# ParBLiSS/FastANI

Measured on AMD Instinct MI355X. Metric: ANI pairs/sec, many-to-many NxN ~5 Mbp genomes, higher is better.
Workload: dtype u32

## Files before the change

### fastani_amd/csrc/kernels/common.hpp

```cpp
#pragma once
#include <hip/hip_runtime.h>
#include <stdint.h>

#if defined(__HIP_DEVICE_COMPILE__)
#define ANI_CONSUME(x) asm volatile("" : "+v"(x))
#else
#define ANI_CONSUME(x) (void)(x)
#endif

namespace ani {

constexpr int kWave = 64;
constexpr int kTPB = 256;
constexpr uint32_t kMurmurSeed = 42;
constexpr uint32_t kSingleNone = 0xffffffffu;

constexpr int kStatStripes = 32;
constexpr int kStatStripeWords = 24;
__device__ __forceinline__ unsigned long long *stat_slot(unsigned long long *base) { return base + (blockIdx.x & (kStatStripes - 1)) * kStatStripeWords; }

constexpr int kPoolStripes = 64, kPoolStripeWords = 16;
constexpr unsigned long long kPoolOverflowBit = 1ull << 63;
__device__ __forceinline__ unsigned long long pool_take(unsigned long long *cursors, uint32_t stripeCap, unsigned long long n)
{
  const uint32_t r = blockIdx.x & (kPoolStripes - 1);
  const unsigned long long off = n ? atomicAdd(&cursors[r * kPoolStripeWords], n) : 0ull;
  return ((unsigned long long)r * stripeCap + off) | (off + n > (unsigned long long)stripeCap ? kPoolOverflowBit : 0ull);
}

__host__ __device__ __forceinline__ uint64_t rotl64(uint64_t x, int r)
{
#if defined(__HIP_DEVICE_COMPILE__)
  uint32_t lo = (uint32_t)x, hi = (uint32_t)(x >> 32);
  if (r >= 32) { const uint32_t t = lo; lo = hi; hi = t; r -= 32; }
  if (r == 0) return ((uint64_t)hi << 32) | lo;
  const uint32_t nh = __builtin_amdgcn_alignbit(hi, lo, 32 - r), nl = __builtin_amdgcn_alignbit(lo, hi, 32 - r);
  return ((uint64_t)nh << 32) | nl;
#else
  return (x << r) | (x >> (64 - r));
#endif
}

__host__ __device__ __forceinline__ uint64_t xorshr33(uint64_t z)
{
  const uint32_t hi = (uint32_t)(z >> 32);
  return ((uint64_t)hi << 32) | ((uint32_t)z ^ (hi >> 1));
}
__host__ __device__ __forceinline__ uint64_t fmix64(uint64_t z)
{
  z = xorshr33(z); z *= 0xff51afd7ed558ccdULL;
  z = xorshr33(z); z *= 0xc4ceb9fe1a85ec53ULL;
  return xorshr33(z);
}

__host__ __device__ __forceinline__ uint32_t murmur32_k16(uint64_t k1, uint64_t k2)
{
  const uint64_t c1 = 0x87c37b91114253d5ULL, c2 = 0x4cf5ad432745937fULL;
  uint64_t h1 = kMurmurSeed, h2 = kMurmurSeed;
  k1 *= c1; k1 = rotl64(k1, 31); k1 *= c2; h1 ^= k1;
  h1 = rotl64(h1, 27); h1 += h2; h1 = h1 * 5 + 0x52dce729;
  k2 *= c2; k2 = rotl64(k2, 33); k2 *= c1; h2 ^= k2;
  h2 = rotl64(h2, 31); h2 += h1; h2 = h2 * 5 + 0x38495ab5;
  h1 ^= 16; h2 ^= 16;
  h1 += h2; h2 += h1;
  h1 = fmix64(h1); h2 = fmix64(h2);
  return (uint32_t)(h1 + h2);
}

__host__ __device__ __forceinline__ uint32_t murmur32_tail(uint64_t k1, uint64_t k2, int k)
{
  const uint64_t c1 = 0x87c37b91114253d5ULL, c2 = 0x4cf5ad432745937fULL;
  uint64_t h1 = kMurmurSeed, h2 = kMurmurSeed;
  if (k > 8) { k2 *= c2; k2 = rotl64(k2, 33); k2 *= c1; h2 ^= k2; }
  k1 *= c1; k1 = rotl64(k1, 31); k1 *= c2; h1 ^= k1;
  h1 ^= (uint64_t)k; h2 ^= (uint64_t)k;
  h1 += h2; h2 += h1;
  h1 = fmix64(h1); h2 = fmix64(h2);
  return (uint32_t)(h1 + h2);
}

__host__ __device__ __forceinline__ uint32_t perm_b32(uint32_t hi, uint32_t lo, uint32_t sel)
{
#if defined(__HIP_DEVICE_COMPILE__)
  return __builtin_amdgcn_perm(hi, lo, sel);
#else
  const uint64_t src = ((uint64_t)hi << 32) | lo;
  uint32_t r = 0;
  for (int i = 0; i < 4; i++) r |= (uint32_t)((src >> (8 * ((sel >> (8 * i)) & 7u))) & 0xffu) << (8 * i);
  return r;
#endif
}
__host__ __device__ __forceinline__ uint32_t alignbyte(uint32_t hi, uint32_t lo, uint32_t n)
{
#if defined(__HIP_DEVICE_COMPILE__)
  return __builtin_amdgcn_alignbyte(hi, lo, n);
#else
  return (uint32_t)(((((uint64_t)hi << 32) | lo) >> (8 * (n & 3u))) & 0xffffffffu);
#endif
}
__host__ __device__ __forceinline__ uint32_t spread_codes4(uint32_t c8)
{
  const uint32_t t = (c8 | (c8 << 12)) & 0x000F000Fu;
  return (t | (t << 6)) & 0x03030303u;
}

__host__ __device__ __forceinline__ uint32_t code_to_ascii(uint32_t c) { return (0x54474341u >> (8 * c)) & 0xffu; }
__host__ __device__ __forceinline__ uint32_t code_to_ascii_comp(uint32_t c) { return (0x41434754u >> (8 * c)) & 0xffu; }
__host__ __device__ __forceinline__ uint32_t ascii_comp(uint32_t b)
{
  return b == 'A' ? 'T' : b == 'C' ? 'G' : b == 'G' ? 'C' : b == 'T' ? 'A' : b;
}
__host__ __device__ __forceinline__ uint32_t ascii_upper(uint32_t b) { return (b > 96 && b < 123) ? b - 32 : b; }

__device__ __forceinline__ int wave_incl_scan(int v)
{
  const int lane = threadIdx.x & (kWave - 1);
#pragma unroll
  for (int d = 1; d < kWave; d <<= 1) {
    int o = __shfl_up(v, d);
    if (lane >= d) v += o;
  }
  return v;
}

__device__ __forceinline__ int wave_incl_scan_dpp(int v)
{
#if defined(__HIP_DEVICE_COMPILE__)
  v += __builtin_amdgcn_update_dpp(0, v, 0x111, 0xf, 0xf, false);
  v += __builtin_amdgcn_update_dpp(0, v, 0x112, 0xf, 0xf, false);
  v += __builtin_amdgcn_update_dpp(0, v, 0x114, 0xf, 0xf, false);
  v += __builtin_amdgcn_update_dpp(0, v, 0x118, 0xf, 0xf, false);
  v += __builtin_amdgcn_update_dpp(0, v, 0x142, 0xa, 0xf, false);
  v += __builtin_amdgcn_update_dpp(0, v, 0x143, 0xc, 0xf, false);
  return v;
#else
  return wave_incl_scan(v);
#endif
}

__device__ __forceinline__ void block_barrier()
{
#if defined(__HIP_DEVICE_COMPILE__)
  asm volatile("s_waitcnt lgkmcnt(0)" ::: "memory");
#endif
  __syncthreads();
}
__device__ __forceinline__ void block_barrier_mem()
{
#if defined(__HIP_DEVICE_COMPILE__)
  asm volatile("s_waitcnt vmcnt(0) lgkmcnt(0)" ::: "memory");
#endif
  __syncthreads();
}

#if defined(__HIP_DEVICE_COMPILE__)
__device__ __forceinline__ uint32_t wave_uniform(uint32_t x) { return (uint32_t)__builtin_amdgcn_readfirstlane((int)x); }
#else
__device__ __forceinline__ uint32_t wave_uniform(uint32_t x) { return x; }
#endif
__device__ __forceinline__ int32_t wave_uniform(int32_t x) { return (int32_t)wave_uniform((uint32_t)x); }
#if defined(__HIP_DEVICE_COMPILE__)
__device__ __forceinline__ int32_t lane_value(int32_t x, int l) { return __builtin_amdgcn_readlane(x, l); }
#else
__device__ __forceinline__ int32_t lane_value(int32_t x, int l) { return __shfl(x, l); }
#endif
__device__ __forceinline__ uint64_t wave_uniform(uint64_t x) { return (uint64_t)wave_uniform((uint32_t)x) | ((uint64_t)wave_uniform((uint32_t)(x >> 32))
    << 32); }

__device__ __forceinline__ int block_excl_scan(int v, int *ws, int *total)
{
  const int lane = threadIdx.x & (kWave - 1), wv = threadIdx.x >> 6;
  int incl = wave_incl_scan(v);
  block_barrier();
  if (lane == kWave - 1) ws[wv] = incl;
  block_barrier();
  int base = 0, tot = 0;
#pragma unroll
  for (int i = 0; i < kTPB / kWave; i++) { int x = ws[i]; if (i < wv) base += x; tot += x; }
  *total = wave_uniform(tot);
  return base + incl - v;
}

__device__ __forceinline__ int block_incl_maxscan(int v, int *ws)
{
  const int lane = threadIdx.x & (kWave - 1), wv = threadIdx.x >> 6;
#pragma unroll
  for (int d = 1; d < kWave; d <<= 1) {
    int o = __shfl_up(v, d);
    if (lane >= d) v = o > v ? o : v;
  }
  block_barrier();
  if (lane == kWave - 1) ws[wv] = v;
  block_barrier();
#pragma unroll
  for (int i = 0; i < kTPB / kWave; i++) { int x = ws[i]; if (i < wv) v = x > v ? x : v; }
  return v;
}

__device__ inline int block_array_excl_scan(int *a, int n, int *ws)
{
  int carry = 0;
  for (int base = 0; base < n; base += kTPB * 8) {
    int first = base + (int)threadIdx.x * 8;
    int loc[8]; int sum = 0;
#pragma unroll
    for (int j = 0; j < 8; j++) { int idx = first + j; int x = idx < n ? a[idx] : 0; loc[j] = sum; sum += x; }
    int tot; int off = block_excl_scan(sum, ws, &tot);
#pragma unroll
    for (int j = 0; j < 8; j++) { int idx = first + j; if (idx < n) a[idx] = carry + off + loc[j]; }
    carry += tot;
  }
  block_barrier_mem();
  return carry;
}

#if defined(__HIP_DEVICE_COMPILE__)
#define ANI_WAVE_SYNC() do { __builtin_amdgcn_fence(__ATOMIC_RELEASE, "wavefront"); __builtin_amdgcn_wave_barrier(); \
    __builtin_amdgcn_fence(__ATOMIC_ACQUIRE, "wavefront"); } while (0)
#else
#define ANI_WAVE_SYNC() (void)__ballot(1)
#endif

template <class K>
__device__ __forceinline__ void bitonic_ce(K &x, K &y, bool up) { if ((x > y) == up) { const K t = x; x = y; y = t; } }

template <class K>
__device__ __forceinline__ void bitonic_quad(K *a, int q, int h, int stride, int size)
{
  const int i0 = ((q & ~(h - 1)) << 2) | (q & (h - 1));
  const bool up = ((i0 & size) == 0);
  K x0 = a[i0], x1 = a[i0 + h], x2 = a[i0 + stride], x3 = a[i0 + stride + h];
  bitonic_ce(x0, x2, up); bitonic_ce(x1, x3, up);
  bitonic_ce(x0, x1, up); bitonic_ce(x2, x3, up);
  a[i0] = x0; a[i0 + h] = x1; a[i0 + stride] = x2; a[i0 + stride + h] = x3;
}

template <class K>
__device__ inline void block_bitonic_sort(K *a, int n2)
{
  constexpr int kWaves = kTPB / kWave;
  const int lane = threadIdx.x & (kWave - 1), wv = threadIdx.x >> 6;
  const int seg = n2 > kWaves * kWave ? n2 / kWaves : n2;
  const bool mine = wv * seg < n2;
  block_barrier();
  for (int size = 2; size <= n2; size <<= 1) {
    int stride = size >> 1;
    while (stride >= 2) {
      const int h = stride >> 1;
      if (stride >= seg) {
        block_barrier();
        for (int q = threadIdx.x; q < (n2 >> 2); q += kTPB) bitonic_quad(a, q, h, stride, size);
        block_barrier();
      } else if (mine) {
        ANI_WAVE_SYNC();
        for (int q = wv * (seg >> 2) + lane; q < (wv + 1) * (seg >> 2); q += kWave) bitonic_quad(a, q, h, stride, size);
      }
      stride >>= 2;
    }
    if (stride == 1) {
      if (seg < 2) {
        block_barrier();
      }
      if (mine) {
        ANI_WAVE_SYNC();
        for (int t = wv * (seg >> 1) + lane; t < (wv + 1) * (seg >> 1); t += kWave) {
          const int lo = 2 * t;
          const bool up = ((lo & size) == 0);
          K x = a[lo], y = a[lo + 1];
          if ((x > y) == up) { a[lo] = y; a[lo + 1] = x; }
        }
      }
    }
  }
  block_barrier();
}

template <int M> __device__ __forceinline__ uint32_t lane_xor(uint32_t x)
{
#if defined(__HIP_DEVICE_COMPILE__)
  if constexpr (M == 1) return (uint32_t)__builtin_amdgcn_mov_dpp((int)x, 0xB1, 0xf, 0xf, true);
  else if constexpr (M == 2) return (uint32_t)__builtin_amdgcn_mov_dpp((int)x, 0x4E, 0xf, 0xf, true);
  else if constexpr (M == 4) {
    int r = __builtin_amdgcn_update_dpp(0, (int)x, 0x104, 0xf, 0x5, false);
    return (uint32_t)__builtin_amdgcn_update_dpp(r, (int)x, 0x114, 0xf, 0xA, false);
  }
  else if constexpr (M == 8) return (uint32_t)__builtin_amdgcn_mov_dpp((int)x, 0x128, 0xf, 0xf, true);
  else if constexpr (M == 16) {
    const auto r = __builtin_amdgcn_permlane16_swap(x, x, false, false);
    return (threadIdx.x & 16) ? r[0] : r[1];
  } else {
    const auto r = __builtin_amdgcn_permlane32_swap(x, x, false, false);
    return (threadIdx.x & 32) ? r[0] : r[1];
  }
#else
  return __shfl_xor(x, M);
#endif
}
template <int M> __device__ __forceinline__ uint64_t lane_xor(uint64_t x)
{
#if !defined(__HIP_DEVICE_COMPILE__)
  return __shfl_xor(x, M);
#endif
  return ((uint64_t)lane_xor<M>((uint32_t)(x >> 32)) << 32) | lane_xor<M>((uint32_t)x);
}

template <class K> __device__ __forceinline__ K sort_pick(K own, K partner, bool keepMin) { return ((partner < own) == keepMin) ? partner : own; }

template <class K, int KPT, int M> __device__ __forceinline__ void sort_lane_stage(K (&k)[KPT], bool keepMin)
{
#pragma unroll
  for (int r = 0; r < KPT; r++) k[r] = sort_pick(k[r], lane_xor<M>(k[r]), keepMin);
}
template <class K, int KPT> __device__ __forceinline__ void sort_thread_merge(K (&k)[KPT], bool up)
{
#pragma unroll
  for (int st = KPT >> 1; st >= 1; st >>= 1)
#pragma unroll
    for (int r = 0; r < KPT; r++)
      if ((r & st) == 0) bitonic_ce(k[r], k[r + st], up);
}

template <class K, int KPT, int WAVES>
__device__ __forceinline__ void block_sort_regs(K *a)
{
  constexpr int NT = kWave * WAVES;
  const int t = threadIdx.x;
  if (WAVES == 1 && t >= kWave) return;
  K k[KPT];
#pragma unroll
  for (int r = 0; r < KPT; r++) k[r] = a[r * NT + t];
  if (WAVES > 1) block_barrier();
#pragma unroll
  for (int size = 2; size <= KPT; size <<= 1)
#pragma unroll
    for (int st = size >> 1; st >= 1; st >>= 1)
#pragma unroll
      for (int r = 0; r < KPT; r++)
        if ((r & st) == 0) bitonic_ce(k[r], k[r + st], size < KPT ? (r & size) == 0 : (t & 1) == 0);
  for (int ts = 2; ts <= NT; ts <<= 1) {
    const bool up = (t & ts) == 0;
    for (int m = ts >> 1; m >= 1; m >>= 1) {
      const bool keepMin = ((t & m) == 0) == up;
      if (WAVES > 1 && m >= kWave) {
#pragma unroll
        for (int r = 0; r < KPT; r++) a[r * NT + t] = k[r];
        block_barrier();
#pragma unroll
        for (int r = 0; r < KPT; r++) k[r] = sort_pick(k[r], a[r * NT + (t ^ m)], keepMin);
        block_barrier();
      } else {
        switch (m) {
          case 32: sort_lane_stage<K, KPT, 32>(k, keepMin); break;
          case 16: sort_lane_stage<K, KPT, 16>(k, keepMin); break;
          case 8: sort_lane_stage<K, KPT, 8>(k, keepMin); break;
          case 4: sort_lane_stage<K, KPT, 4>(k, keepMin); break;
          case 2: sort_lane_stage<K, KPT, 2>(k, keepMin); break;
          default: sort_lane_stage<K, KPT, 1>(k, keepMin); break;
        }
      }
    }
    sort_thread_merge<K, KPT>(k, up);
  }
#pragma unroll
  for (int r = 0; r < KPT; r++) a[t * KPT + r] = k[r];
}

template <class K, int KPT> __device__ __forceinline__ void wave_sort_regs(K (&k)[KPT])
{
  const int lane = threadIdx.x & (kWave - 1);
#pragma unroll
  for (int size = 2; size <= KPT; size <<= 1)
#pragma unroll
    for (int st = size >> 1; st >= 1; st >>= 1)
#pragma unroll
      for (int r = 0; r < KPT; r++)
        if ((r & st) == 0) bitonic_ce(k[r], k[r + st], size < KPT ? (r & size) == 0 : (lane & 1) == 0);
  for (int ts = 2; ts <= kWave; ts <<= 1) {
    const bool up = (lane & ts) == 0;
    for (int m = ts >> 1; m >= 1; m >>= 1) {
      const bool keepMin = ((lane & m) == 0) == up;
      switch (m) {
        case 32: sort_lane_stage<K, KPT, 32>(k, keepMin); break;
        case 16: sort_lane_stage<K, KPT, 16>(k, keepMin); break;
        case 8: sort_lane_stage<K, KPT, 8>(k, keepMin); break;
        case 4: sort_lane_stage<K, KPT, 4>(k, keepMin); break;
        case 2: sort_lane_stage<K, KPT, 2>(k, keepMin); break;
        default: sort_lane_stage<K, KPT, 1>(k, keepMin); break;
      }
    }
    sort_thread_merge<K, KPT>(k, up);
  }
}

constexpr int kBlockSortMax = 4096;
__host__ __device__ __forceinline__ int next_pow2_dev(int n) { int p = 1; while (p < n) p <<= 1; return p; }
template <class K>
__device__ __forceinline__ void block_sort(K *a, int n)
{
  int n2 = next_pow2_dev(n); n2 = n2 < kWave ? kWave : n2;
  for (int i = n + (int)threadIdx.x; i < n2; i += kTPB) a[i] = (K)~(K)0;
#ifdef ANI_SORT_LDS
  block_bitonic_sort<K>(a, n2);
  return;
#endif
  block_barrier();
  switch (n2) {
    case 64: block_sort_regs<K, 1, 1>(a); break;
    case 128: block_sort_regs<K, 2, 1>(a); break;
    case 256: block_sort_regs<K, 4, 1>(a); break;
    case 512: block_sort_regs<K, 2, kTPB / kWave>(a); break;
    case 1024: block_sort_regs<K, 4, kTPB / kWave>(a); break;
    case 2048: block_sort_regs<K, 8, kTPB / kWave>(a); break;
    case 4096: block_sort_regs<K, 16, kTPB / kWave>(a); break;
    default: __builtin_trap();
  }
  block_barrier();
}

__device__ __forceinline__ int xcd_item(int block, int gridBlocks) { return (block & 7) * (gridBlocks >> 3) + (block >> 3); }
__host__ __device__ __forceinline__ unsigned pad8(size_t n) { return (unsigned)((n + 7) / 8 * 8); }

__host__ __device__ __forceinline__ int next_pow2(int n) { int p = 1; while (p < n) p <<= 1; return p; }

}
```

### fastani_amd/csrc/kernels/sketch.hpp

```cpp
#pragma once
#include "common.hpp"

namespace ani {

constexpr int kPer = 12;
constexpr int kTile = kTPB * kPer;
constexpr uint64_t kSkipKey = ~0ull;

struct TileDesc {
  int32_t contig;
  int32_t firstPos;
};
struct TileMeta {
  uint32_t off;
  int32_t cnt;
  int32_t firstP;
  int32_t lastP;
};

__device__ __forceinline__ void hash_positions_packed16(const uint32_t *wds, int32_t len, int32_t i0, int local0, uint64_t (&key)[kPer])
{
  const int32_t nWords = (len + 15) >> 4;
  const int32_t w0 = i0 >> 4;
  const int sh = (i0 & 15) * 2;
  const uint64_t a = w0 < nWords ? wds[w0] : 0u, b = w0 + 1 < nWords ? wds[w0 + 1] : 0u, c = w0 + 2 < nWords ? wds[w0 + 2] : 0u;
  const uint64_t lo = a | (b << 32);
  const uint64_t bits = sh ? ((lo >> sh) | (c << (64 - sh))) : lo;
  uint32_t F[7], R[7];
#pragma unroll
  for (int d = 0; d < 7; d++) {
    const uint32_t c8 = (uint32_t)(bits >> (8 * d)) & 0xffu;
    const uint32_t sp = spread_codes4(c8);
    F[d] = perm_b32(0u, 0x54474341u, sp);
    R[6 - d] = perm_b32(0u, 0x41434754u, perm_b32(0u, sp, 0x00010203u));
  }
  const int32_t nPos = len - 16 + 1;
#pragma unroll
  for (int j = 0; j < kPer; j++) {
    uint32_t f[4], r[4];
    const int fq = j >> 2, fr = j & 3, rq = (12 - j) >> 2, rr = (12 - j) & 3;
#pragma unroll
    for (int t = 0; t < 4; t++) {
      f[t] = fr ? alignbyte(F[fq + t + 1], F[fq + t], (uint32_t)fr) : F[fq + t];
      r[t] = rr ? alignbyte(R[rq + t + 1], R[rq + t], (uint32_t)rr) : R[rq + t];
    }
    const uint32_t hf = murmur32_k16(((uint64_t)f[1] << 32) | f[0], ((uint64_t)f[3] << 32) | f[2]);
    const uint32_t hb = murmur32_k16(((uint64_t)r[1] << 32) | r[0], ((uint64_t)r[3] << 32) | r[2]);
    const bool ok = (i0 + j < nPos) && (hf != hb);
    const uint32_t h = hf < hb ? hf : hb;
    key[j] = ok ? (((uint64_t)h << 32) | (uint32_t)(kTile - 1 - (local0 + j))) : kSkipKey;
  }
}

template <bool PACKED>
__device__ __forceinline__ void hash_positions(const void *seq, int64_t off, int32_t len, int32_t i0, int local0,
                                               int k, uint64_t (&key)[kPer])
{
  if (PACKED && k == 16) { hash_positions_packed16((const uint32_t *)seq + off, len, i0, local0, key); return; }
  uint64_t bits = 0;
  const uint8_t *bytes = nullptr;
  if (PACKED) {
    const uint32_t *wds = (const uint32_t *)seq + off;
    const int32_t nWords = (len + 15) >> 4;
    const int32_t w0 = i0 >> 4;
    const int sh = (i0 & 15) * 2;
    uint64_t a = w0 < nWords ? wds[w0] : 0u;
    uint64_t b = w0 + 1 < nWords ? wds[w0 + 1] : 0u;
    uint64_t c = w0 + 2 < nWords ? wds[w0 + 2] : 0u;
    uint64_t lo = a | (b << 32);
    bits = sh ? ((lo >> sh) | (c << (64 - sh))) : lo;
  } else {
    bytes = (const uint8_t *)seq + off;
  }
  auto fwd_byte = [&](int j) -> uint64_t {
    if (PACKED) return code_to_ascii((uint32_t)(bits >> (2 * j)) & 3u);
    int32_t p = i0 + j;
    return p < len ? ascii_upper(bytes[p]) : 0u;
  };
  auto rc_byte = [&](int j) -> uint64_t {
    if (PACKED) return code_to_ascii_comp((uint32_t)(bits >> (2 * j)) & 3u);
    int32_t p = i0 + j;
    return p < len ? ascii_comp(ascii_upper(bytes[p])) : 0u;
  };

  uint64_t flo = 0, fhi = 0, rlo = 0, rhi = 0;
#pragma unroll
  for (int j = 0; j < 8; j++) {
    flo |= fwd_byte(j) << (8 * j);
    fhi |= fwd_byte(8 + j) << (8 * j);
    rhi |= rc_byte(j) << (8 * (7 - j));
    rlo |= rc_byte(8 + j) << (8 * (7 - j));
  }
  const bool k16 = (k == 16);
  const uint64_t maskLo = k >= 8 ? ~0ull : ((1ull << (8 * k)) - 1);
  const uint64_t maskHi = k16 ? ~0ull : (k > 8 ? ((1ull << (8 * (k - 8))) - 1) : 0ull);
  const int rsh = 8 * (16 - k);
  const int32_t nPos = len - k + 1;

#pragma unroll
  for (int j = 0; j < kPer; j++) {
    uint32_t hf, hb;
    if (k16) {
      hf = murmur32_k16(flo, fhi);
      hb = murmur32_k16(rlo, rhi);
    } else {
      uint64_t r1, r2;
      if (rsh < 64) { r1 = (rlo >> rsh) | (rhi << (64 - rsh)); r2 = rhi >> rsh; }
      else { r1 = rsh == 64 ? rhi : (rhi >> (rsh - 64)); r2 = 0; }
      hf = murmur32_tail(flo & maskLo, fhi & maskHi, k);
      hb = murmur32_tail(r1, r2, k);
    }
    const bool ok = (i0 + j < nPos) && (hf != hb);
    const uint32_t h = hf < hb ? hf : hb;
    key[j] = ok ? (((uint64_t)h << 32) | (uint32_t)(kTile - 1 - (local0 + j))) : kSkipKey;
    const uint64_t nb = fwd_byte(16 + j), nc = rc_byte(16 + j);
    flo = (flo >> 8) | (fhi << 56);
    fhi = (fhi >> 8) | (nb << 56);
    rhi = (rhi << 8) | (rlo >> 56);
    rlo = (rlo << 8) | nc;
  }
}

__device__ __forceinline__ void tile_winnow_keys(const uint64_t (&key)[kPer], int32_t B, int32_t nPos, int w, int lo, int hiEmit,
                                                 uint64_t *keys, int *ws,
                                                 uint64_t (&W)[kPer], bool (&em)[kPer], int &tileFirstP, int &tileLastP)
{
  const int t = threadIdx.x;
  const int local0 = t * kPer;
  bool own_ok[kPer];
  if (t == 0) ws[kTPB + 8] = -1;
  if (w >= kPer && w <= 4 * kPer) {
    uint64_t suf = kSkipKey, pre = kSkipKey;
#pragma unroll
    for (int j = kPer - 1; j >= 0; j--) { suf = key[j] < suf ? key[j] : suf; keys[local0 + j] = suf; }
#pragma unroll
    for (int j = 0; j < kPer; j++) { own_ok[j] = key[j] != kSkipKey; pre = key[j] < pre ? key[j] : pre; W[j] = pre; }
    block_barrier();
    const int aHi = (w - 1) / kPer;
    uint64_t allHi = kSkipKey, allLo = kSkipKey;
#pragma unroll
    for (int x = 1; x <= 3; x++) {
      if (x <= aHi) {
        const uint64_t v = t - x >= 0 ? keys[(t - x) * kPer] : kSkipKey;
        allLo = allHi; allHi = v < allHi ? v : allHi;
      }
    }
    int a = aHi, b = (w - 1) - aHi * kPer;
#pragma unroll
    for (int j = 0; j < kPer; j++) {
      const uint64_t whole = a == aHi ? allHi : allLo;
      const int tb = t - a - 1;
      const uint64_t part = (b > 0 && tb >= 0) ? keys[tb * kPer + kPer - b] : kSkipKey;
      uint64_t m = whole < part ? whole : part;
      W[j] = m < W[j] ? m : W[j];
      if (b == 0) { a--; b = kPer - 1; } else b--;
    }
  } else {
#pragma unroll
  for (int j = 0; j < kPer; j++) { keys[local0 + j] = key[j]; W[j] = key[j]; own_ok[j] = key[j] != kSkipKey; }

  int p = 1;
  while (2 * p <= w) {
    block_barrier();
    uint64_t r[kPer];
#pragma unroll
    for (int j = 0; j < kPer; j++) { int q = local0 + j - p; r[j] = q >= 0 ? keys[q] : kSkipKey; }
    block_barrier();
#pragma unroll
    for (int j = 0; j < kPer; j++) { W[j] = r[j] < W[j] ? r[j] : W[j]; keys[local0 + j] = W[j]; }
    p <<= 1;
  }
  block_barrier();
  if (w > p) {
    const int d = w - p;
#pragma unroll
    for (int j = 0; j < kPer; j++) { int q = local0 + j - d; uint64_t r = q >= 0 ? keys[q] : kSkipKey; W[j] = r < W[j] ? r : W[j]; }
  }
  }

  int P[kPer]; bool val[kPer];
  int myMax = -1, myFirst = -1;
#pragma unroll
  for (int j = 0; j < kPer; j++) {
    const int l = local0 + j;
    val[j] = own_ok[j] && l >= lo + w - 1 && l < hiEmit && (B + l) < nPos;
    P[j] = val[j] ? (kTile - 1 - (int)(uint32_t)W[j]) : -1;
    if (val[j]) { if (myFirst < 0) myFirst = P[j]; myMax = P[j]; }
  }
  const int lane = t & (kWave - 1), wv = t >> 6;
  int v = myMax;
#pragma unroll
  for (int d = 1; d < kWave; d <<= 1) { const int o = __shfl_up(v, d); if (lane >= d) v = o > v ? o : v; }
  int prev = __shfl_up(v, 1); if (lane == 0) prev = -1;
  if (lane == kWave - 1) ws[wv] = v;
  block_barrier();
  int lastAll = -1;
#pragma unroll
  for (int i = 0; i < kTPB / kWave; i++) { const int x = ws[i]; if (i < wv) prev = x > prev ? x : prev; lastAll = x > lastAll ? x : lastAll; }
  if (myFirst >= 0 && prev < 0) ws[kTPB + 8] = myFirst;
  block_barrier();
  const int firstAll = ws[kTPB + 8];
#pragma unroll
  for (int j = 0; j < kPer; j++) {
    em[j] = val[j] && P[j] != prev;
    if (val[j]) prev = P[j];
  }
  tileFirstP = firstAll >= 0 ? B + firstAll : -1;
  tileLastP = lastAll >= 0 ? B + lastAll : -1;
  block_barrier();
}

template <bool PACKED>
__device__ __forceinline__ void tile_winnow(const void *seq, int64_t off, int32_t len, int32_t B, int k, int w,
                                            uint64_t *keys, int *ws,
                                            uint64_t (&W)[kPer], bool (&em)[kPer], int &tileFirstP, int &tileLastP)
{
  uint64_t key[kPer];
  hash_positions<PACKED>(seq, off, len, B + (int)threadIdx.x * kPer, (int)threadIdx.x * kPer, k, key);
  tile_winnow_keys(key, B, len - k + 1, w, 0, kTile, keys, ws, W, em, tileFirstP, tileLastP);
}

static __global__ __launch_bounds__(kTPB) void k_sketch_tiles(const uint32_t *__restrict__ packed, const uint8_t *__restrict__ ascii,
                                                       const int64_t *__restrict__ contigOff, const int32_t *__restrict__ contigLen,
                                                       const uint8_t *__restrict__ contigMode ,
                                                       const TileDesc *__restrict__ tiles, int k, int w,
                                                       uint32_t *__restrict__ poolHash, int32_t *__restrict__ poolWpos,
                                                       uint32_t poolCap, unsigned long long *__restrict__ poolCount,
                                                       TileMeta *__restrict__ meta)
{
  __shared__ uint64_t keys[kTile];
  __shared__ int ws[kTPB + 16];
  __shared__ unsigned long long sBase;
  const TileDesc td = tiles[blockIdx.x];
  const int64_t off = contigOff[td.contig];
  const int32_t len = contigLen[td.contig];
  uint64_t W[kPer]; bool em[kPer]; int firstP, lastP;
  if (contigMode[td.contig]) tile_winnow<true>(packed, off, len, td.firstPos, k, w, keys, ws, W, em, firstP, lastP);
  else tile_winnow<false>(ascii, off, len, td.firstPos, k, w, keys, ws, W, em, firstP, lastP);
  int cnt = 0;
#pragma unroll
  for (int j = 0; j < kPer; j++) cnt += em[j];
  int total; int rank = block_excl_scan(cnt, ws, &total);
  if (threadIdx.x == 0) sBase = pool_take(poolCount, poolCap, (unsigned long long)total);
  block_barrier();
  const unsigned long long base = sBase & ~kPoolOverflowBit;
  if (!(sBase & kPoolOverflowBit)) {
#pragma unroll
    for (int j = 0; j < kPer; j++)
      if (em[j]) {
        poolHash[base + rank] = (uint32_t)(W[j] >> 32);
        poolWpos[base + rank] = td.firstPos + (int)threadIdx.x * kPer + j - w + 1;
        rank++;
      }
  }
  if (threadIdx.x == 0) {
    TileMeta m; m.off = (uint32_t)base; m.cnt = total; m.firstP = firstP; m.lastP = lastP;
    meta[blockIdx.x] = m;
  }
}

__device__ __forceinline__ int32_t owner_of(const uint32_t *__restrict__ start, int32_t nContigs, uint32_t u)
{
  int32_t lo = 0, hi = nContigs;
  while (hi - lo > 1) { int32_t mid = (lo + hi) >> 1; if (start[mid] <= u) lo = mid; else hi = mid; }
  return lo;
}

static __global__ void k_expand_tiles(const uint32_t *__restrict__ tileStart, int32_t nContigs, uint32_t nTiles, int32_t stride, TileDesc *__restrict__ tiles)
{
  const uint32_t T = blockIdx.x * blockDim.x + threadIdx.x;
  if (T >= nTiles) return;
  const int32_t c = owner_of(tileStart, nContigs, T);
  tiles[T] = TileDesc{c, (int32_t)((T - tileStart[c]) * (uint32_t)stride)};
}

static __global__ void k_sketch_tile_counts(const TileDesc *__restrict__ tiles, const TileMeta *__restrict__ meta, int nTiles,
                                     int32_t *__restrict__ outCnt , uint8_t *__restrict__ dropFirst)
{
  int T = blockIdx.x * blockDim.x + threadIdx.x;
  if (T >= nTiles) return;
  const TileMeta m = meta[T];
  int drop = 0;
  if (m.cnt > 0) {
    const int c = tiles[T].contig;
    for (int U = T - 1; U >= 0 && tiles[U].contig == c; U--) {
      const int lp = meta[U].lastP;
      if (lp >= 0) { drop = (lp == m.firstP); break; }
    }
  }
  dropFirst[T] = (uint8_t)drop;
  outCnt[T] = m.cnt - drop;
}

static __global__ __launch_bounds__(kTPB) void k_sketch_gather(const TileDesc *__restrict__ tiles, const TileMeta *__restrict__ meta,
                                                        const uint8_t *__restrict__ dropFirst, const uint32_t *__restrict__ outOff,
                                                        const uint32_t *__restrict__ poolHash, const int32_t *__restrict__ poolWpos,
                                                        int32_t seqIdBase, uint32_t *__restrict__ records )
{
  const int T = blockIdx.x;
  const TileMeta m = meta[T];
  const int drop = dropFirst[T];
  const int n = m.cnt - drop;
  const size_t dst = outOff[T];
  const int32_t seqId = seqIdBase + tiles[T].contig;
  for (int r = threadIdx.x; r < n; r += blockDim.x) {
    const uint32_t src = m.off + drop + r;
    uint32_t *rec = records + 3 * (dst + r);
    rec[0] = poolHash[src]; rec[1] = (uint32_t)seqId; rec[2] = (uint32_t)poolWpos[src];
  }
}

struct FragDesc {
  int32_t contig;
  int32_t start;
};

static __global__ void k_expand_frags(const uint32_t *__restrict__ fragStart, const int32_t *__restrict__ contigGenomeLocal,
                               const int32_t *__restrict__ contigQSeqBase, int32_t nContigs, uint32_t nFrags, int32_t fragLen,
                               FragDesc *__restrict__ frags, int32_t *__restrict__ fragGenome, int32_t *__restrict__ fragQSeq)
{
  const uint32_t f = blockIdx.x * blockDim.x + threadIdx.x;
  if (f >= nFrags) return;
  const int32_t c = owner_of(fragStart, nContigs, f);
  const int32_t i = (int32_t)(f - fragStart[c]);
  frags[f] = FragDesc{c, i * fragLen};
  fragGenome[f] = contigGenomeLocal[c];
  fragQSeq[f] = contigQSeqBase[c] + i;
}

constexpr int kFragHashCap = 4096;
static_assert(kFragHashCap <= kBlockSortMax, "block_sort (common.hpp) sorts at most kBlockSortMax keys");

template <bool PACKED>
__device__ __forceinline__ void fragment_sketch_body(const void *__restrict__ seq, const int64_t *__restrict__ contigOff,
                                                     const FragDesc *__restrict__ frags, int fragLen, int k, int w,
                                                     uint32_t *__restrict__ pool, uint32_t poolCap,
                                                     unsigned long long *__restrict__ poolCount,
                                                     uint32_t *__restrict__ fragOff, int32_t *__restrict__ fragS,
                                                     int *__restrict__ maxS,
                                                     uint64_t *keys, uint32_t *hbuf, int *ws, unsigned long long *sBasePtr)
{
  const FragDesc fd = frags[blockIdx.x];
  const int64_t off = contigOff[fd.contig];
  const int32_t vlen = fd.start + fragLen;
  const int32_t nPos = fragLen - k + 1;
  const int stride = kTile - (w - 1);
  int produced = 0;
  int prevLastP = -1;
  bool overflow = false;
  for (int32_t B = 0; B == 0 || B + (w - 1) < nPos; B += stride) {
    uint64_t W[kPer]; bool em[kPer]; int firstP, lastP;
    tile_winnow<PACKED>(seq, off, vlen, fd.start + B, k, w, keys, ws, W, em, firstP, lastP);
    int cnt = 0;
#pragma unroll
    for (int j = 0; j < kPer; j++) cnt += em[j];
    int total; int rank = block_excl_scan(cnt, ws, &total);
    const int drop = (total > 0 && prevLastP >= 0 && firstP == prevLastP) ? 1 : 0;
#pragma unroll
    for (int j = 0; j < kPer; j++)
      if (em[j]) {
        const int r = produced + rank - drop;
        if (rank >= drop) { if (r < kFragHashCap) hbuf[r] = (uint32_t)(W[j] >> 32); }
        rank++;
      }
    produced += total - drop;
    if (produced > kFragHashCap) { overflow = true; produced = kFragHashCap; }
    if (lastP >= 0) prevLastP = lastP;
    block_barrier();
  }
  const int n = produced;
  block_sort<uint32_t>(hbuf, n);
  const int per = (n + kTPB - 1) / kTPB;
  const int lo = threadIdx.x * per, hi = lo + per < n ? lo + per : n;
  int cntU = 0;
  for (int i = lo; i < hi; i++) cntU += (i == 0 || hbuf[i] != hbuf[i - 1]);
  int s; int r = block_excl_scan(cntU, ws, &s);
  if (threadIdx.x == 0) {
    *sBasePtr = pool_take(poolCount, poolCap, (unsigned long long)s);
    fragOff[blockIdx.x] = (uint32_t)*sBasePtr;
    fragS[blockIdx.x] = overflow ? -1 : s;
    atomicMax((int *)stat_slot((unsigned long long *)maxS), overflow ? 0x7fffffff : s);
  }
  block_barrier();
  const unsigned long long base = *sBasePtr & ~kPoolOverflowBit;
  if (!(*sBasePtr & kPoolOverflowBit))
    for (int i = lo; i < hi; i++)
      if (i == 0 || hbuf[i] != hbuf[i - 1]) pool[base + r++] = hbuf[i];
}

template <bool SINGLE>
static __global__ __launch_bounds__(kTPB, SINGLE ? 4 : 3) void k_fragment_sketch(const uint32_t *__restrict__ packed, const uint8_t *__restrict__ ascii,
                                                          const int64_t *__restrict__ contigOff, const uint8_t *__restrict__ contigMode,
                                                          const FragDesc *__restrict__ frags, int fragLen, int k, int w,
                                                          uint32_t *__restrict__ pool, uint32_t poolCap, unsigned long long *__restrict__ poolCount,
                                                          uint32_t *__restrict__ fragOff, int32_t *__restrict__ fragS, int *__restrict__ maxS)
{
  __shared__ uint64_t keys[kTile];
  __shared__ uint32_t hbufOwn[SINGLE ? 1 : kFragHashCap];
  __shared__ int ws[kTPB + 16];
  __shared__ unsigned long long sBase;
  static_assert(kFragHashCap * 4 <= kTile * 8, "staging buffer fits the key array");
  uint32_t *hbuf = SINGLE ? (uint32_t *)keys : hbufOwn;
  if (contigMode[frags[blockIdx.x].contig])
    fragment_sketch_body<true>(packed, contigOff, frags, fragLen, k, w, pool, poolCap, poolCount, fragOff, fragS, maxS, keys, hbuf, ws, &sBase);
  else
    fragment_sketch_body<false>(ascii, contigOff, frags, fragLen, k, w, pool, poolCap, poolCount, fragOff, fragS, maxS, keys, hbuf, ws, &sBase);
}

struct FusedInfo {
  int32_t frag;
  int32_t emitEnd;
  int32_t fragLocal0;
};

static __global__ void k_expand_fused(const uint32_t *__restrict__ tileStart, const uint32_t *__restrict__ fragStart, int32_t nContigs, uint32_t nTiles,
                               int32_t fragLen, int32_t w, int32_t stride, TileDesc *__restrict__ tiles, FusedInfo *__restrict__ info)
{
  const uint32_t T = blockIdx.x * blockDim.x + threadIdx.x;
  if (T >= nTiles) return;
  const int32_t c = owner_of(tileStart, nContigs, T);
  const int32_t t = (int32_t)(T - tileStart[c]);
  const int32_t nFragC = (int32_t)(fragStart[c + 1] - fragStart[c]);
  if (t < nFragC) {
    const int32_t B = t == 0 ? 0 : t * fragLen - (w - 1);
    tiles[T] = TileDesc{c, B};
    info[T] = FusedInfo{(int32_t)fragStart[c] + t, t * fragLen - B + fragLen, t * fragLen - B};
  } else {
    const int32_t base = nFragC > 0 ? nFragC * fragLen - (w - 1) : 0;
    tiles[T] = TileDesc{c, base + (t - nFragC) * stride};
    info[T] = FusedInfo{-1, kTile, 0};
  }
}

__device__ __forceinline__ void fragment_finish(uint32_t *hbuf, int n, bool overflow, int frag, uint32_t *__restrict__ pool, uint32_t poolCap,
                                                unsigned long long *__restrict__ poolCount, uint32_t *__restrict__ fragOff, int32_t *__restrict__ fragS,
                                                int *__restrict__ maxS, int *ws, unsigned long long *sBasePtr)
{
  block_sort<uint32_t>(hbuf, n);
  const int per = (n + kTPB - 1) / kTPB;
  const int lo = threadIdx.x * per, hi = lo + per < n ? lo + per : n;
  int cntU = 0;
  for (int i = lo; i < hi; i++) cntU += (i == 0 || hbuf[i] != hbuf[i - 1]);
  int s; int r = block_excl_scan(cntU, ws, &s);
  if (threadIdx.x == 0) {
    *sBasePtr = pool_take(poolCount, poolCap, (unsigned long long)s);
    fragOff[frag] = (uint32_t)*sBasePtr;
    fragS[frag] = overflow ? -1 : s;
    atomicMax((int *)stat_slot((unsigned long long *)maxS), overflow ? 0x7fffffff : s);
  }
  block_barrier();
  const unsigned long long base = *sBasePtr & ~kPoolOverflowBit;
  if (!(*sBasePtr & kPoolOverflowBit))
    for (int i = lo; i < hi; i++)
      if (i == 0 || hbuf[i] != hbuf[i - 1]) pool[base + r++] = hbuf[i];
}

static __global__ void k_pack_fragment_pool(const uint32_t *__restrict__ pool, uint32_t *__restrict__ fragOff, const int32_t *__restrict__ s,
    const uint32_t *__restrict__ newOff,
                                     uint32_t nFrag, uint32_t *__restrict__ out)
{
  const uint32_t f = (uint32_t)(((uint64_t)blockIdx.x * blockDim.x + threadIdx.x) >> 6), lane = threadIdx.x & 63;
  if (f >= nFrag) return;
  const uint32_t src = fragOff[f], dst = newOff[f];
  const int n = s[f];
  for (int i = (int)lane; i < n; i += 64) out[dst + i] = pool[src + i];
  ANI_WAVE_SYNC();
  if (lane == 0) fragOff[f] = dst;
}

static __global__ void k_fragset_rebase(uint32_t n, const uint32_t *__restrict__ srcOff, const int32_t *__restrict__ srcS,
    const int32_t *__restrict__ srcGenome,
                                        const int32_t *__restrict__ srcQSeq, uint32_t addOff, int32_t addGenome,
                                        uint32_t *__restrict__ dstOff, int32_t *__restrict__ dstS, int32_t *__restrict__ dstGenome,
                                            int32_t *__restrict__ dstQSeq)
{
  for (uint32_t i = blockIdx.x * blockDim.x + threadIdx.x; i < n; i += gridDim.x * blockDim.x) {
    dstOff[i] = srcOff[i] + addOff; dstS[i] = srcS[i]; dstGenome[i] = srcGenome[i] + addGenome; dstQSeq[i] = srcQSeq[i];
  }
}

template <bool PACKED>
__device__ __forceinline__ void fused_tile_body(const void *__restrict__ seq, int64_t off, int32_t len, const TileDesc td, const FusedInfo fi, int k, int w,
    int fragLen,
                                                uint32_t *__restrict__ poolHash, int32_t *__restrict__ poolWpos, uint32_t poolCap,
                                                    unsigned long long *__restrict__ poolCount,
                                                TileMeta *__restrict__ meta,
                                                uint32_t *__restrict__ qPool, uint32_t qCap, unsigned long long *__restrict__ qCount,
                                                uint32_t *__restrict__ fragOff, int32_t *__restrict__ fragS, int *__restrict__ maxS,
                                                uint64_t *keys, int *ws, unsigned long long *sBasePtr)
{
  const int local0 = (int)threadIdx.x * kPer;
  uint64_t key[kPer];
  hash_positions<PACKED>(seq, off, len, td.firstPos + local0, local0, k, key);
  uint64_t W[kPer]; bool em[kPer]; int firstP, lastP;
  tile_winnow_keys(key, td.firstPos, len - k + 1, w, 0, fi.emitEnd, keys, ws, W, em, firstP, lastP);
  {
    int cnt = 0;
#pragma unroll
    for (int j = 0; j < kPer; j++) cnt += em[j];
    int total; int rank = block_excl_scan(cnt, ws, &total);
    if (threadIdx.x == 0) *sBasePtr = pool_take(poolCount, poolCap, (unsigned long long)total);
    block_barrier();
    const unsigned long long base = *sBasePtr & ~kPoolOverflowBit;
    if (!(*sBasePtr & kPoolOverflowBit)) {
#pragma unroll
      for (int j = 0; j < kPer; j++)
        if (em[j]) {
          poolHash[base + rank] = (uint32_t)(W[j] >> 32);
          poolWpos[base + rank] = td.firstPos + local0 + j - w + 1;
          rank++;
        }
    }
    if (threadIdx.x == 0) { TileMeta m; m.off = (uint32_t)base; m.cnt = total; m.firstP = firstP; m.lastP = lastP; meta[blockIdx.x] = m; }
  }
  if (fi.frag < 0) return;
  const int f0 = fi.fragLocal0, fEnd = f0 + fragLen - k;
  bool inR[kPer]; int myFirst = 0x7fffffff;
#pragma unroll
  for (int j = 0; j < kPer; j++) {
    const int l = local0 + j;
    inR[j] = key[j] != kSkipKey && l >= f0 + w - 1 && l <= fEnd;
    if (inR[j] && l < myFirst) myFirst = l;
  }
#pragma unroll
  for (int d = 32; d > 0; d >>= 1) { const int o = __shfl_down(myFirst, d); myFirst = o < myFirst ? o : myFirst; }
  block_barrier();
  if ((threadIdx.x & (kWave - 1)) == 0) ws[threadIdx.x >> 6] = myFirst;
  block_barrier();
  int firstL = 0x7fffffff;
#pragma unroll
  for (int i = 0; i < kTPB / kWave; i++) { const int x = ws[i]; firstL = x < firstL ? x : firstL; }
  uint32_t *hbuf = (uint32_t *)keys;
  int cnt = 0;
#pragma unroll
  for (int j = 0; j < kPer; j++) { inR[j] = inR[j] && (em[j] || local0 + j == firstL); cnt += inR[j]; }
  int total; int rank = block_excl_scan(cnt, ws, &total);
#pragma unroll
  for (int j = 0; j < kPer; j++)
    if (inR[j]) { if (rank < kFragHashCap) hbuf[rank] = (uint32_t)(W[j] >> 32); rank++; }
  const bool overflow = total > kFragHashCap;
  block_barrier();
  fragment_finish(hbuf, overflow ? kFragHashCap : total, overflow, fi.frag, qPool, qCap, qCount, fragOff, fragS, maxS, ws, sBasePtr);
}

static __global__ __launch_bounds__(kTPB, 3) void k_sketch_fused(const uint32_t *__restrict__ packed, const uint8_t *__restrict__ ascii,
                                                          const int64_t *__restrict__ contigOff, const int32_t *__restrict__ contigLen,
                                                              const uint8_t *__restrict__ contigMode,
                                                          const TileDesc *__restrict__ tiles, const FusedInfo *__restrict__ info, int k, int w, int fragLen,
                                                          uint32_t *__restrict__ poolHash, int32_t *__restrict__ poolWpos, uint32_t poolCap,
                                                              unsigned long long *__restrict__ poolCount,
                                                          TileMeta *__restrict__ meta,
                                                          uint32_t *__restrict__ qPool, uint32_t qCap, unsigned long long *__restrict__ qCount,
                                                          uint32_t *__restrict__ fragOff, int32_t *__restrict__ fragS, int *__restrict__ maxS)
{
  __shared__ uint64_t keys[kTile];
  __shared__ int ws[kTPB + 16];
  __shared__ unsigned long long sBase;
  const TileDesc td = tiles[blockIdx.x];
  const FusedInfo fi = info[blockIdx.x];
  const int64_t off = contigOff[td.contig];
  const int32_t len = contigLen[td.contig];
  if (contigMode[td.contig])
    fused_tile_body<true>(packed, off, len, td, fi, k, w, fragLen, poolHash, poolWpos, poolCap, poolCount, meta, qPool, qCap, qCount, fragOff, fragS, maxS,
        keys, ws, &sBase);
  else
    fused_tile_body<false>(ascii, off, len, td, fi, k, w, fragLen, poolHash, poolWpos, poolCap, poolCount, meta, qPool, qCap, qCount, fragOff, fragS, maxS,
        keys, ws, &sBase);
}

}
```

Baseline: 5.526 million.

## Use DPP wave scans and remove block barriers in sketch winnowing

Replaces shuffle-based wave max and prefix scans with DPP-based max, min and sum scans. Computes the tile's first winnow position through a min-scan, which removes a shared-memory race slot and two block barriers from tile_winnow_keys. The fragment path is restructured to use a single scan plus one barrier, with the forced first element appended at the end. Also folds constants into the murmur multiply-add, makes pool base wave-uniform and uses byte-offset stores. This changes the fragment hash order and relies on the callers' later barriers for correctness, so there is some reordering and race risk.

```diff
diff --git a/fastani_amd/csrc/kernels/common.hpp b/fastani_amd/csrc/kernels/common.hpp
--- a/fastani_amd/csrc/kernels/common.hpp
+++ b/fastani_amd/csrc/kernels/common.hpp
@@ -53,14 +53,20 @@
   return xorshr33(z);
 }
 
+__host__ __device__ __forceinline__ uint64_t mul5_add(uint64_t x, uint32_t c)
+{
+  const uint64_t addend = ((uint64_t)((uint32_t)(x >> 32) * 5u) << 32) | c;
+  return (uint64_t)(uint32_t)x * 5u + addend;
+}
+
 __host__ __device__ __forceinline__ uint32_t murmur32_k16(uint64_t k1, uint64_t k2)
 {
   const uint64_t c1 = 0x87c37b91114253d5ULL, c2 = 0x4cf5ad432745937fULL;
   uint64_t h1 = kMurmurSeed, h2 = kMurmurSeed;
   k1 *= c1; k1 = rotl64(k1, 31); k1 *= c2; h1 ^= k1;
-  h1 = rotl64(h1, 27); h1 += h2; h1 = h1 * 5 + 0x52dce729;
+  h1 = rotl64(h1, 27); h1 = mul5_add(h1, 5u * kMurmurSeed + 0x52dce729u);
   k2 *= c2; k2 = rotl64(k2, 33); k2 *= c1; h2 ^= k2;
-  h2 = rotl64(h2, 31); h2 += h1; h2 = h2 * 5 + 0x38495ab5;
+  h2 = rotl64(h2, 31); h2 += h1; h2 = mul5_add(h2, 0x38495ab5);
   h1 ^= 16; h2 ^= 16;
   h1 += h2; h2 += h1;
   h1 = fmix64(h1); h2 = fmix64(h2);
@@ -138,6 +144,37 @@
 #endif
 }
 
+__device__ __forceinline__ int wave_incl_maxscan_dpp(int v)
+{
+#if defined(__HIP_DEVICE_COMPILE__)
+  constexpr int lowest = (int)0x80000000;
+#define ANI_DPP_MAX_STEP(ctrl, rows) { const int o = __builtin_amdgcn_update_dpp(lowest, v, ctrl, rows, 0xf, false); v = o > v ? o : v; }
+  ANI_DPP_MAX_STEP(0x111, 0xf) ANI_DPP_MAX_STEP(0x112, 0xf) ANI_DPP_MAX_STEP(0x114, 0xf) ANI_DPP_MAX_STEP(0x118, 0xf)
+  ANI_DPP_MAX_STEP(0x142, 0xa) ANI_DPP_MAX_STEP(0x143, 0xc)
+#undef ANI_DPP_MAX_STEP
+  return v;
+#else
+  const int lane = threadIdx.x & (kWave - 1);
+  for (int d = 1; d < kWave; d <<= 1) { const int o = __shfl_up(v, d); if (lane >= d) v = o > v ? o : v; }
+  return v;
+#endif
+}
+__device__ __forceinline__ int wave_incl_minscan_dpp(int v)
+{
+#if defined(__HIP_DEVICE_COMPILE__)
+  constexpr int highest = 0x7fffffff;
+#define ANI_DPP_MIN_STEP(ctrl, rows) { const int o = __builtin_amdgcn_update_dpp(highest, v, ctrl, rows, 0xf, false); v = o < v ? o : v; }
+  ANI_DPP_MIN_STEP(0x111, 0xf) ANI_DPP_MIN_STEP(0x112, 0xf) ANI_DPP_MIN_STEP(0x114, 0xf) ANI_DPP_MIN_STEP(0x118, 0xf)
+  ANI_DPP_MIN_STEP(0x142, 0xa) ANI_DPP_MIN_STEP(0x143, 0xc)
+#undef ANI_DPP_MIN_STEP
+  return v;
+#else
+  const int lane = threadIdx.x & (kWave - 1);
+  for (int d = 1; d < kWave; d <<= 1) { const int o = __shfl_up(v, d); if (lane >= d) v = o < v ? o : v; }
+  return v;
+#endif
+}
+
 __device__ __forceinline__ void block_barrier()
 {
 #if defined(__HIP_DEVICE_COMPILE__)
@@ -170,7 +207,7 @@
 __device__ __forceinline__ int block_excl_scan(int v, int *ws, int *total)
 {
   const int lane = threadIdx.x & (kWave - 1), wv = threadIdx.x >> 6;
-  int incl = wave_incl_scan(v);
+  int incl = wave_incl_scan_dpp(v);
   block_barrier();
   if (lane == kWave - 1) ws[wv] = incl;
   block_barrier();
diff --git a/fastani_amd/csrc/kernels/sketch.hpp b/fastani_amd/csrc/kernels/sketch.hpp
--- a/fastani_amd/csrc/kernels/sketch.hpp
+++ b/fastani_amd/csrc/kernels/sketch.hpp
@@ -121,14 +121,13 @@
   }
 }
 
-__device__ __forceinline__ void tile_winnow_keys(const uint64_t (&key)[kPer], int32_t B, int32_t nPos, int w, int lo, int hiEmit,
+__device__ __forceinline__ void tile_winnow_keys(const uint64_t (&key)[kPer], int32_t B, int w, int lo, int hiEmit,
                                                  uint64_t *keys, int *ws,
                                                  uint64_t (&W)[kPer], bool (&em)[kPer], int &tileFirstP, int &tileLastP)
 {
   const int t = threadIdx.x;
   const int local0 = t * kPer;
   bool own_ok[kPer];
-  if (t == 0) ws[kTPB + 8] = -1;
   if (w >= kPer && w <= 4 * kPer) {
     uint64_t suf = kSkipKey, pre = kSkipKey;
 #pragma unroll
@@ -178,36 +177,36 @@
   }
   }
 
-  int P[kPer]; bool val[kPer];
-  int myMax = -1, myFirst = -1;
+  int P[kPer];
+  int myMax = -1; uint32_t firstU = ~0u;
 #pragma unroll
   for (int j = 0; j < kPer; j++) {
     const int l = local0 + j;
-    val[j] = own_ok[j] && l >= lo + w - 1 && l < hiEmit && (B + l) < nPos;
-    P[j] = val[j] ? (kTile - 1 - (int)(uint32_t)W[j]) : -1;
-    if (val[j]) { if (myFirst < 0) myFirst = P[j]; myMax = P[j]; }
-  }
+    const bool val = own_ok[j] && l >= lo + w - 1 && l < hiEmit;
+    P[j] = val ? (kTile - 1 - (int)(uint32_t)W[j]) : -1;
+    myMax = P[j] > myMax ? P[j] : myMax;
+    firstU = (uint32_t)P[j] < firstU ? (uint32_t)P[j] : firstU;
+  }
+  const int myFirst = (int)(firstU & 0x7fffffffu);
   const int lane = t & (kWave - 1), wv = t >> 6;
-  int v = myMax;
-#pragma unroll
-  for (int d = 1; d < kWave; d <<= 1) { const int o = __shfl_up(v, d); if (lane >= d) v = o > v ? o : v; }
+  const int v = wave_incl_maxscan_dpp(myMax), vF = wave_incl_minscan_dpp(myFirst);
   int prev = __shfl_up(v, 1); if (lane == 0) prev = -1;
-  if (lane == kWave - 1) ws[wv] = v;
-  block_barrier();
-  int lastAll = -1;
-#pragma unroll
-  for (int i = 0; i < kTPB / kWave; i++) { const int x = ws[i]; if (i < wv) prev = x > prev ? x : prev; lastAll = x > lastAll ? x : lastAll; }
-  if (myFirst >= 0 && prev < 0) ws[kTPB + 8] = myFirst;
-  block_barrier();
-  const int firstAll = ws[kTPB + 8];
+  if (lane == kWave - 1) { ws[wv] = v; ws[8 + wv] = vF; }
+  block_barrier();
+  int lastAll = -1, firstAll = 0x7fffffff;
+#pragma unroll
+  for (int i = 0; i < kTPB / kWave; i++) {
+    const int x = ws[i], y = ws[8 + i];
+    if (i < wv) prev = x > prev ? x : prev;
+    lastAll = x > lastAll ? x : lastAll; firstAll = y < firstAll ? y : firstAll;
+  }
 #pragma unroll
   for (int j = 0; j < kPer; j++) {
-    em[j] = val[j] && P[j] != prev;
-    if (val[j]) prev = P[j];
-  }
-  tileFirstP = firstAll >= 0 ? B + firstAll : -1;
+    em[j] = P[j] > prev;
+    prev = P[j] > prev ? P[j] : prev;
+  }
+  tileFirstP = firstAll != 0x7fffffff ? B + firstAll : -1;
   tileLastP = lastAll >= 0 ? B + lastAll : -1;
-  block_barrier();
 }
 
 template <bool PACKED>
@@ -217,7 +216,7 @@
 {
   uint64_t key[kPer];
   hash_positions<PACKED>(seq, off, len, B + (int)threadIdx.x * kPer, (int)threadIdx.x * kPer, k, key);
-  tile_winnow_keys(key, B, len - k + 1, w, 0, kTile, keys, ws, W, em, tileFirstP, tileLastP);
+  tile_winnow_keys(key, B, w, 0, kTile, keys, ws, W, em, tileFirstP, tileLastP);
 }
 
 static __global__ __launch_bounds__(kTPB) void k_sketch_tiles(const uint32_t *__restrict__ packed, const uint8_t *__restrict__ ascii,
@@ -243,14 +242,18 @@
   int total; int rank = block_excl_scan(cnt, ws, &total);
   if (threadIdx.x == 0) sBase = pool_take(poolCount, poolCap, (unsigned long long)total);
   block_barrier();
-  const unsigned long long base = sBase & ~kPoolOverflowBit;
-  if (!(sBase & kPoolOverflowBit)) {
+  const unsigned long long sb = wave_uniform((uint64_t)sBase);
+  const unsigned long long base = sb & ~kPoolOverflowBit;
+  if (!(sb & kPoolOverflowBit)) {
+    char *const hp = (char *)(poolHash + base), *const wp = (char *)(poolWpos + base);
+    uint32_t ob = (uint32_t)rank * 4u;
+    const int32_t wpos0 = td.firstPos + (int)threadIdx.x * kPer - w + 1;
 #pragma unroll
     for (int j = 0; j < kPer; j++)
       if (em[j]) {
-        poolHash[base + rank] = (uint32_t)(W[j] >> 32);
-        poolWpos[base + rank] = td.firstPos + (int)threadIdx.x * kPer + j - w + 1;
-        rank++;
+        *(uint32_t *)(hp + ob) = (uint32_t)(W[j] >> 32);
+        *(int32_t *)(wp + ob) = wpos0 + j;
+        ob += 4u;
       }
   }
   if (threadIdx.x == 0) {
@@ -493,7 +496,7 @@
   uint64_t key[kPer];
   hash_positions<PACKED>(seq, off, len, td.firstPos + local0, local0, k, key);
   uint64_t W[kPer]; bool em[kPer]; int firstP, lastP;
-  tile_winnow_keys(key, td.firstPos, len - k + 1, w, 0, fi.emitEnd, keys, ws, W, em, firstP, lastP);
+  tile_winnow_keys(key, td.firstPos, w, 0, fi.emitEnd, keys, ws, W, em, firstP, lastP);
   {
     int cnt = 0;
 #pragma unroll
@@ -501,46 +504,58 @@
     int total; int rank = block_excl_scan(cnt, ws, &total);
     if (threadIdx.x == 0) *sBasePtr = pool_take(poolCount, poolCap, (unsigned long long)total);
     block_barrier();
-    const unsigned long long base = *sBasePtr & ~kPoolOverflowBit;
-    if (!(*sBasePtr & kPoolOverflowBit)) {
+    const unsigned long long sb = wave_uniform((uint64_t)*sBasePtr);
+    const unsigned long long base = sb & ~kPoolOverflowBit;
+    if (!(sb & kPoolOverflowBit)) {
+      char *const hp = (char *)(poolHash + base), *const wp = (char *)(poolWpos + base);
+      uint32_t ob = (uint32_t)rank * 4u;
+      const int32_t wpos0 = td.firstPos + local0 - w + 1;
 #pragma unroll
       for (int j = 0; j < kPer; j++)
         if (em[j]) {
-          poolHash[base + rank] = (uint32_t)(W[j] >> 32);
-          poolWpos[base + rank] = td.firstPos + local0 + j - w + 1;
-          rank++;
+          *(uint32_t *)(hp + ob) = (uint32_t)(W[j] >> 32);
+          *(int32_t *)(wp + ob) = wpos0 + j;
+          ob += 4u;
         }
     }
     if (threadIdx.x == 0) { TileMeta m; m.off = (uint32_t)base; m.cnt = total; m.firstP = firstP; m.lastP = lastP; meta[blockIdx.x] = m; }
   }
   if (fi.frag < 0) return;
   const int f0 = fi.fragLocal0, fEnd = f0 + fragLen - k;
-  bool inR[kPer]; int myFirst = 0x7fffffff;
+  bool inR[kPer]; int myFirst = 0x7fffffff, cnt = 0;
 #pragma unroll
   for (int j = 0; j < kPer; j++) {
     const int l = local0 + j;
     inR[j] = key[j] != kSkipKey && l >= f0 + w - 1 && l <= fEnd;
     if (inR[j] && l < myFirst) myFirst = l;
-  }
-#pragma unroll
-  for (int d = 32; d > 0; d >>= 1) { const int o = __shfl_down(myFirst, d); myFirst = o < myFirst ? o : myFirst; }
-  block_barrier();
-  if ((threadIdx.x & (kWave - 1)) == 0) ws[threadIdx.x >> 6] = myFirst;
-  block_barrier();
-  int firstL = 0x7fffffff;
-#pragma unroll
-  for (int i = 0; i < kTPB / kWave; i++) { const int x = ws[i]; firstL = x < firstL ? x : firstL; }
+    cnt += inR[j] && em[j];
+  }
+  const int lane = (int)threadIdx.x & (kWave - 1), wv = (int)threadIdx.x >> 6;
+  const int incl = wave_incl_scan_dpp(cnt), vF = wave_incl_minscan_dpp(myFirst);
+  if (lane == kWave - 1) { ws[wv] = incl; ws[8 + wv] = vF; }
+  if (threadIdx.x == 0) ws[16] = 0;
+  block_barrier();
+  int rank = incl - cnt, emitted = 0, firstL = 0x7fffffff;
+#pragma unroll
+  for (int i = 0; i < kTPB / kWave; i++) {
+    const int x = ws[i], y = ws[8 + i];
+    if (i < wv) rank += x;
+    emitted += x; firstL = y < firstL ? y : firstL;
+  }
+  emitted = wave_uniform(emitted);
   uint32_t *hbuf = (uint32_t *)keys;
-  int cnt = 0;
-#pragma unroll
-  for (int j = 0; j < kPer; j++) { inR[j] = inR[j] && (em[j] || local0 + j == firstL); cnt += inR[j]; }
-  int total; int rank = block_excl_scan(cnt, ws, &total);
 #pragma unroll
   for (int j = 0; j < kPer; j++)
-    if (inR[j]) { if (rank < kFragHashCap) hbuf[rank] = (uint32_t)(W[j] >> 32); rank++; }
-  const bool overflow = total > kFragHashCap;
-  block_barrier();
-  fragment_finish(hbuf, overflow ? kFragHashCap : total, overflow, fi.frag, qPool, qCap, qCount, fragOff, fragS, maxS, ws, sBasePtr);
+    if (inR[j] && em[j]) hbuf[rank++] = (uint32_t)(W[j] >> 32);
+  if (myFirst == firstL && firstL != 0x7fffffff) {
+#pragma unroll
+    for (int j = 0; j < kPer; j++)
+      if (local0 + j == firstL && !em[j]) { hbuf[emitted] = (uint32_t)(W[j] >> 32); ws[16] = 1; }
+  }
+  block_barrier();
+  static_assert(kTile <= kFragHashCap, "one tile's positions cannot overflow the staging buffer");
+  const int total = emitted + wave_uniform(ws[16]);
+  fragment_finish(hbuf, total, false, fi.frag, qPool, qCap, qCount, fragOff, fragS, maxS, ws, sBasePtr);
 }
 
 static __global__ __launch_bounds__(kTPB, 3) void k_sketch_fused(const uint32_t *__restrict__ packed, const uint8_t *__restrict__ ascii,
```

Result: faster. 5.636 million, median of 6 (+2.0%).
